# Elliotshui/ABRSimulator

Hardware: AMD Instinct MI355X
Metric: env_steps_per_sec (higher is better)
Workload: dtype f64

## Files before the change

### abrsimulator_amd/csrc/abr_env.hip

```cpp
#include <hip/hip_runtime.h>

#include <climits>
#include <cmath>
#include <cstdarg>
#include <cstdio>
#include <cstdlib>
#include <cstring>
#include <new>
#include <type_traits>
#include <vector>

#include "abr_env.h"

#ifdef ABR_SPLIT_STAMPS
#include "abr_diag_stamps.h"
#else
#define ABR_STAMP(n)
#define ABR_STAMP_INIT()
#define ABR_STAMP_FLUSH()
#define ABR_WG_TIME(slot)
#define ABR_WG_WHERE(role)
#define K3_STAMP_DECL
#define K3_STAMP(n)
#define K3_STAMP_FLUSH()
// ... 496 lines not shown
            const bool hit = dling && (dl2 >= target);
            done_dl = done_dl || hit;
            chunk_id += hit ? 1 : 0;
            avail_k = hit ? avail_next : avail_k;
            const double bufA = hit ? buf + L : buf;
            const bool playing = running && !(be || su);
            sk += playing ? (uint32_t)k : 0u;
            n_play += playing ? 1 : 0;
            const double bufB = playing ? bufA - sd : bufA;
            bf = bufB >= max_buffer;
            be = bufB <= 0.0;
            buf = be ? 0.0 : bufB;
            su = su && !(buf >= sul);
            k += running ? 1 : 0;
            const bool next = running && (chunk_id < V) && (k < max_ticks);
            n_su += (next && su) ? 1 : 0;
            n_rb += (next && !su && be) ? 1 : 0;
            const bool call = done_dl && (k >= avail_k) && !bf;
            running = next && !call;
            const bool cross = (k == k_end);
            c = cross ? c_next : c;
            crossed = crossed || cross;
        }
        if (active) {
            s.buf = buf; s.dl = dl; s.c = c; s.k = k; s.chunk_id = chunk_id; s.n_su = n_su;
            s.n_rb = n_rb; s.n_play = n_play; s.n_dl = n_dl; s.avail_k = avail_k;
            s.su = su; s.be = be; s.bf = bf; s.done_dl = done_dl; s.running = running;
            s.sumk += (long long)sk;
            (void)crossed;
        }
    }

    if (touched) {
        lane_store(s, p, i);
        p.n_su_obs[i] = n_su_obs; p.n_rb_obs[i] = n_rb_obs; p.episode_no[i] = episode_no;
        p.last_bw[i] = last_bw; p.hist_n[i] = hist_n; p.hist_s[i] = hist_s; p.var_run[i] = var_run;
        p.done[i] = done;
        if (MODE != 0) {
            for (int32_t t = step_idx; t < n_total; t++) {
                const int64_t o = (int64_t)t * p.n_lanes + i;
                if (reward_out) reward_out[o] = 0.0f;
                if (done_out) done_out[o] = done;
                if ((MODE == 2 || MODE == 4) && actions_out) actions_out[o] = -1;
                if (obs_out)
                    write_obs(s, p, i, obs_out + (int64_t)t * ABR_OBS_DIM * p.n_lanes, last_bw);
            }
        }
    }
}

using abrx::LaneJ;

template <bool SPEEDS>
struct SpeedParams;
template <>
struct SpeedParams<true> {
    static __device__ __forceinline__ const double *lane_speeds(const EnvParams &p) { return p.lane_speeds; }
    static __device__ __forceinline__ int32_t speed_rows(const EnvParams &p) { return p.speed_rows; }
    static __device__ __forceinline__ double *sd_lane(const EnvParams &p) { return p.sd_lane; }
    static __device__ __forceinline__ double *pt_lane(const EnvParams &p) { return p.pt_lane; }
    static __device__ __forceinline__ double *pt_sum(const EnvParams &p) { return p.pt_sum; }
    static __device__ __forceinline__ int32_t *pl_left(const EnvParams &p) { return p.pl_left; }
    static __device__ __forceinline__ int32_t *play_id(const EnvParams &p) { return p.play_id; }
};
template <>
struct SpeedParams<false> {
    static __device__ __forceinline__ constexpr const double *lane_speeds(const EnvParams &) { return nullptr; }
    static __device__ __forceinline__ constexpr int32_t speed_rows(const EnvParams &) { return 1; }
};

template <bool SPEEDS = true, class TB = abrx::TablesT<SPEEDS>>
__device__ inline TB make_tables(const EnvParams &p, bool cascade = true) {
    TB t;
    t.G = p.G; t.interval_tick = p.interval_tick; t.avail_tick = p.avail_tick;
    t.L = p.chunk_length; t.sd = p.sd; t.max_buffer = p.max_buffer;
    t.start_up_length = p.start_up_length; t.V = p.video_length; t.max_ticks = p.max_ticks;
    using SP = SpeedParams<SPEEDS>;
    if constexpr (SPEEDS) {
        t.per_lane_speed = SP::lane_speeds(p) != nullptr;
        t.speed_rows = SP::lane_speeds(p) ? SP::speed_rows(p) : 0;
        t.speed_stride = p.n_lanes; t.speeds = SP::lane_speeds(p);
    }
    t.drain = p.drain;
    if (SP::lane_speeds(p) || !cascade) t.drain.n = 0;
#ifdef ABR_NO_DRAIN_CASCADE
    t.drain.n = 0;
#endif
    return t;
}

template <bool SPEEDS = true>
__device__ inline void lanej_load(LaneJ &s, const EnvParams &p, int64_t i) {
    using SP = SpeedParams<SPEEDS>;
    s.buf = p.buf[i]; s.sumk = p.sumk[i];
    s.k = p.k[i]; s.chunk_id = p.chunk_id[i]; s.n_su = p.n_su[i]; s.n_rb = p.n_rb[i];
    s.n_play = p.n_play[i]; s.cur.j = p.j[i]; s.cur.tpos = p.tpos[i];
    s.last_action = p.last_action[i];
    const uint8_t f = p.flags[i];
    s.su = f & kFlagStartUp; s.be = f & kFlagBufEmpty; s.bf = f & kFlagBufFull;
    const int32_t c = s.chunk_id < p.video_length ? s.chunk_id : p.video_length;
    s.avail_k = p.avail_tick[c];
    if constexpr (SPEEDS) {
        if (SP::lane_speeds(p)) { s.sd = SP::sd_lane(p)[i]; s.pt = SP::pt_lane(p)[i]; } else { s.sd = p.sd; s.pt = 0.0; }
        s.lane = i; s.pl_left = 0; s.play_id = 0; s.pt_sum = 0.0;
        if (SP::lane_speeds(p) && SP::speed_rows(p) >= 2) { s.pl_left = SP::pl_left(p)[i]; s.play_id = SP::play_id(p)[i]; s.pt_sum = SP::pt_sum(p)[i]; }
    } else {
        s.sd = p.sd; s.lane = i;
    }
}

template <bool SPEEDS = true>
__device__ inline void lanej_store(const LaneJ &s, const EnvParams &p, int64_t i) {
    p.buf[i] = s.buf; p.sumk[i] = s.sumk;
    p.k[i] = s.k; p.chunk_id[i] = s.chunk_id; p.n_su[i] = s.n_su; p.n_rb[i] = s.n_rb;
    p.n_play[i] = s.n_play; p.j[i] = s.cur.j; p.tpos[i] = s.cur.tpos; p.last_action[i] = s.last_action;
    p.flags[i] = (uint8_t)((s.su ? kFlagStartUp : 0) | (s.be ? kFlagBufEmpty : 0) |
                           (s.bf ? kFlagBufFull : 0) | kFlagArmed);
    if constexpr (SPEEDS) {
        using SP = SpeedParams<SPEEDS>;
        if (SP::lane_speeds(p)) { SP::sd_lane(p)[i] = s.sd; SP::pt_lane(p)[i] = s.pt; }
        if (SP::lane_speeds(p) && SP::speed_rows(p) >= 2) { SP::pl_left(p)[i] = s.pl_left; SP::play_id(p)[i] = s.play_id; SP::pt_sum(p)[i] = s.pt_sum; }
    }
}

#ifndef ABR_NO_NT_STORES
#define ABR_OUT(ref, val) __builtin_nontemporal_store((val), &(ref))
#else
#define ABR_OUT(ref, val) ((ref) = (val))
#endif

template <bool SPEEDS = true>
__device__ inline void write_obs_j(const LaneJ &s, const EnvParams &p, int64_t i, float *obs,
                                   double last_bw) {
    if (!obs) return;
    const int64_t n = p.n_lanes;
    ABR_OUT(obs[ABR_OBS_CHUNK_ID * n + i], (float)s.chunk_id);
    ABR_OUT(obs[ABR_OBS_LAST_BITRATE * n + i], (float)s.last_action);
    ABR_OUT(obs[ABR_OBS_LAST_BANDWIDTH * n + i], (float)last_bw);
    ABR_OUT(obs[ABR_OBS_BUFFER_LEVEL * n + i], (float)s.buf);
    ABR_OUT(obs[ABR_OBS_GLOBAL_TIME * n + i], (float)p.G[s.k]);
    ABR_OUT(obs[ABR_OBS_PLAY_TIME * n + i], (float)(SpeedParams<SPEEDS>::lane_speeds(p) ? s.pt : p.GP[s.n_play]));
    ABR_OUT(obs[ABR_OBS_REBUFFER_TIME * n + i], (float)p.G[s.n_rb]);
    ABR_OUT(obs[ABR_OBS_STARTUP_TIME * n + i], (float)p.G[s.n_su]);
}

__device__ inline void write_obs_vals(const LaneJ &s, const EnvParams &p, int64_t i, float *obs, double last_bw,
                                      double g_k, double g_play, double g_rb, double g_su) {
    if (!obs) return;
    const int64_t n = p.n_lanes;
    ABR_OUT(obs[ABR_OBS_CHUNK_ID * n + i], (float)s.chunk_id);
    ABR_OUT(obs[ABR_OBS_LAST_BITRATE * n + i], (float)s.last_action);
    ABR_OUT(obs[ABR_OBS_LAST_BANDWIDTH * n + i], (float)last_bw);
    ABR_OUT(obs[ABR_OBS_BUFFER_LEVEL * n + i], (float)s.buf);
    ABR_OUT(obs[ABR_OBS_GLOBAL_TIME * n + i], (float)g_k);
    ABR_OUT(obs[ABR_OBS_PLAY_TIME * n + i], (float)g_play);
    ABR_OUT(obs[ABR_OBS_REBUFFER_TIME * n + i], (float)g_rb);
    ABR_OUT(obs[ABR_OBS_STARTUP_TIME * n + i], (float)g_su);
}

#ifndef ABR_JUMP_WAVES
#define ABR_JUMP_WAVES 5
#endif
#ifndef ABR_JUMP_WAVES_ONE
#define ABR_JUMP_WAVES_ONE 4
#endif
#define ABR_JUMP_BOUNDS(MODE, SAMPLE) \
// ... 288 lines not shown
    L->max_ticks = mt;
    L->n_intervals = (int32_t)n_iv;
    size_t o = 0;
    const size_t A = 256;
    size_t N = (size_t)n_lanes, V = (size_t)c->video_length;
    L->G = o; o = align_up(o + sizeof(double) * ((size_t)mt + 2), A);
    L->GP = o; o = align_up(o + sizeof(double) * ((size_t)mt + 2), A);
    L->interval_tick = o; o = align_up(o + sizeof(int32_t) * ((size_t)L->n_intervals + 8), A);
    L->avail_tick = o; o = align_up(o + sizeof(int32_t) * (V + 2), A);
    L->f64_state = o; o = align_up(o + sizeof(double) * 8 * N, A);
    L->i64_state = o; o = align_up(o + sizeof(long long) * 1 * N, A);
    L->i32_state = o; o = align_up(o + sizeof(int32_t) * 15 * N, A);
    L->u8_state = o; o = align_up(o + 2 * N, A);
    L->action_hist = o; o = align_up(o + V * N, A);
    L->bw_hist = o; o = align_up(o + sizeof(double) * V * N, A);
    L->ep_terms = o; o = align_up(o + sizeof(double) * 4 * N, A);
    L->mpc_action = o; o = align_up(o + sizeof(int32_t) * N, A);
    L->mpc_scratch = o; o = align_up(o + mpc_scratch_bytes_max(N), A);
    L->tag = o; o = align_up(o + sizeof(WorkspaceTag), A);
    L->total = o;
    return ABR_OK;
}

extern "C" int abr_env_workspace_bytes(const abr_env_config *cfg, int64_t n_lanes,
                                       size_t *bytes_out) {
    Layout L;
    int rc = compute_layout(cfg, n_lanes, &L);
    if (rc) return rc;
    if (!bytes_out) return fail(ABR_E_INVALID, "bytes_out is NULL");
    *bytes_out = L.total;
    return ABR_OK;
}

extern "C" int abr_env_create(const abr_env_config *cfg, const double *traces_dev,
                              const int64_t *trace_off_dev, const int32_t *trace_len_dev,
                              int32_t n_traces, int64_t n_lanes, void *workspace_dev,
                              size_t workspace_bytes, void *stream, abr_env **env_out) {
    Layout L;
    int rc = compute_layout(cfg, n_lanes, &L);
    if (rc) return rc;
    if (!env_out) return fail(ABR_E_INVALID, "env_out is NULL");
    if (!traces_dev || !trace_off_dev || !trace_len_dev || n_traces < 1)
        return fail(ABR_E_INVALID, "trace arrays missing");
    if (!workspace_dev || ((uintptr_t)workspace_dev & 255))
        return fail(ABR_E_WORKSPACE, "workspace must be non-NULL and 256-B aligned");
    if (workspace_bytes < L.total)
        return fail(ABR_E_WORKSPACE, "workspace has %zu bytes, need %zu", workspace_bytes, L.total);

    const int32_t mt = L.max_ticks;
    abrx::TickTables tt = abrx::build_tick_tables(cfg->interval, cfg->chunk_length, cfg->speed,
                                                  cfg->video_length, mt, L.n_intervals);
    std::vector<double> &G = tt.G, &GP = tt.GP;
    std::vector<int32_t> &itick = tt.interval_tick, &atick = tt.avail_tick;
    const double sd = tt.sd;
    const int32_t P = tt.play_ticks_per_chunk;
    int32_t t_block = tt.min_interval_ticks < 128 ? tt.min_interval_ticks : 128;
    if (t_block < 1) t_block = 1;
    if (P == INT_MAX)
        return fail(ABR_E_UNSUPPORTED, "max_ticks %d too small to play one chunk", mt);

    abr_env *e = new (std::nothrow) abr_env;
    if (!e) return fail(ABR_E_INVALID, "out of host memory");
    memset(e, 0, sizeof(*e));
    e->cfg = *cfg;
    e->impl = 3;
    e->chains_proven = abrx::chains_proven(itick.data(), itick.size(), mt, sd, cfg->chunk_length, cfg->max_buffer, cfg->ladder,
                                           cfg->n_rates);
    e->workspace_bytes = L.total;
    EnvParams &p = e->p;
    p.n_rates = cfg->n_rates; p.video_length = cfg->video_length; p.max_ticks = mt;
    p.auto_reset = cfg->auto_reset; p.play_ticks_per_chunk = P; p.n_intervals = L.n_intervals;
    p.t_block = t_block; p.n_traces = n_traces;
    p.chunk_length = cfg->chunk_length; p.max_buffer = cfg->max_buffer;
    p.start_up_length = cfg->start_up_length;
    p.wr = cfg->rebuffer_weight; p.wv = cfg->variance_weight; p.ws = cfg->startup_weight;
    p.wl = cfg->latency_weight; p.sd = sd;
    for (int r = 0; r < ABR_MAX_RATES; r++) p.ladder[r] = cfg->ladder[r];
    p.n_lanes = n_lanes; p.lane_id_base = 0;
    char *w = (char *)workspace_dev;
    p.G = (const double *)(w + L.G); p.GP = (const double *)(w + L.GP);
    p.interval_tick = (const int32_t *)(w + L.interval_tick);
    p.avail_tick = (const int32_t *)(w + L.avail_tick);
    p.drain = abrx::make_drain_tab(sd, cfg->max_buffer + cfg->chunk_length);
    p.traces = traces_dev; p.trace_off = trace_off_dev; p.trace_len = trace_len_dev;
    const size_t N = (size_t)n_lanes;
    double *f = (double *)(w + L.f64_state);
    p.buf = f; p.last_bw = f + N; p.hist_n = f + 2 * N; p.hist_s = f + 3 * N;
    p.sd_lane = f + 4 * N; p.pt_lane = f + 5 * N; p.pt_sum = f + 6 * N; p.var_run = f + 7 * N; p.lane_speeds = nullptr;
    p.speed_rows = 1;
    p.speed_rule = abrx::SpeedRuleBlock{};
    p.sumk = (long long *)(w + L.i64_state);
    int32_t *q = (int32_t *)(w + L.i32_state);
    p.k = q; p.chunk_id = q + N; p.n_su = q + 2 * N; p.n_rb = q + 3 * N; p.n_play = q + 4 * N;
    p.j = q + 5 * N; p.tpos = q + 6 * N; p.trace_id = q + 7 * N; p.offset0 = q + 8 * N;
    p.last_action = q + 9 * N; p.n_su_obs = q + 10 * N; p.n_rb_obs = q + 11 * N;
    p.episode_no = q + 12 * N; p.pl_left = q + 13 * N; p.play_id = q + 14 * N;
    uint8_t *u = (uint8_t *)(w + L.u8_state);
    p.flags = u; p.done = u + N;
    p.action_hist = (uint8_t *)(w + L.action_hist);
    p.bw_hist = (double *)(w + L.bw_hist);
    p.ep_qoe_terms = (double *)(w + L.ep_terms);
    e->mpc_action = (int32_t *)(w + L.mpc_action);
    e->mpc_scratch = (void *)(w + L.mpc_scratch);

    hipStream_t st = (hipStream_t)stream;
    hipError_t he;
#define UP(dst, vec)                                                                           \
    he = hipMemcpyAsync((void *)(dst), (vec).data(), (vec).size() * sizeof((vec)[0]),          \
                        hipMemcpyHostToDevice, st);                                            \
    if (he != hipSuccess) { delete e; return fail(ABR_E_HIP, "table upload: %s", hipGetErrorString(he)); }
    UP(p.G, G) UP(p.GP, GP) UP(p.interval_tick, itick) UP(p.avail_tick, atick)
#undef UP
    he = hipMemsetAsync(w + L.f64_state, 0, L.total - L.f64_state, st);
    if (he == hipSuccess) he = hipMemsetAsync(p.done, ABR_DONE_EPISODE, N, st);
    {
        WorkspaceTag &tg = e->tag;
        memset(&tg, 0, sizeof(tg));
        tg.magic = kTagMagic; tg.abi_version = ABR_ABI_VERSION; tg.layout_rev = kLayoutRev; tg.n_rates = (uint32_t)cfg->n_rates;
        tg.n_lanes = n_lanes; tg.video_length = cfg->video_length; tg.max_ticks = mt; tg.n_intervals = L.n_intervals;
        tg.total_bytes = L.total; tg.chunk_length = cfg->chunk_length; tg.interval = cfg->interval; tg.speed = cfg->speed;
        e->tag_dev = w + L.tag;
        if (he == hipSuccess) he = hipMemcpyAsync(e->tag_dev, &tg, sizeof(tg), hipMemcpyHostToDevice, st);
    }
    if (he == hipSuccess) he = hipStreamSynchronize(st);
    if (he != hipSuccess) { delete e; return fail(ABR_E_HIP, "workspace init: %s", hipGetErrorString(he)); }
    *env_out = e;
    return ABR_OK;
}

extern "C" int abr_env_destroy(abr_env *env) {
    delete env;
    return ABR_OK;
}

extern "C" int abr_env_has_impl(int32_t impl) {
    switch (impl) {
    case 0: case 1: case 2: case 3: case 5: return 1;
#ifdef ABR_WITH_ASYNC
    case 4: return 1;
#endif
#ifdef ABR_WITH_RING
    case 6: case 7: return 1;
#endif
    default: return 0;
    }
}

enum Feature { kLaneSpeeds, kSpeedRule, kRuleRollout, kMpcRollout, kPolicyRollout };
static const struct { unsigned impls; const char *what; } kFeatures[] = {
    {0xFDu, "per-lane speeds and speed schedules need the event-driven kernels"},
    {0x2Du, "a speed rule needs the event-driven kernels that read it"},
    {0x0Bu, "rule rollouts run on the one-thread-per-lane kernels"},
    {0xFDu, "the fused MPC rollout needs the event-driven kernels"},
    {0xFDu, "the fused policy rollout needs the event-driven kernels"},
};

static int require(Feature f, int impl) {
    const unsigned ok = kFeatures[f].impls;
    if (ok >> impl & 1u) return ABR_OK;
    int ks[8], n = 0, len = 0;
    for (int k = 0; k < 8; k++)
        if ((ok >> k & 1u) && abr_env_has_impl(k)) ks[n++] = k;
    char list[48] = "";
    for (int i = 0; i < n; i++)
        len += snprintf(list + len, sizeof(list) - len, "%s%d", i == 0 ? "" : i + 1 < n ? ", " : " or ", ks[i]);
    return fail(ABR_E_UNSUPPORTED, "%s (impl %s), not impl %d", kFeatures[f].what, list, impl);
// ... 3439 lines not shown
```

### abrsimulator_amd/csrc/abr_exact_jump.h

```cpp
#ifndef ABR_EXACT_JUMP_H
#define ABR_EXACT_JUMP_H

#include <stdint.h>
#include <string.h>

#if defined(__HIPCC__)
#define ABR_HD __host__ __device__ inline
#else
#define ABR_HD inline
#endif

namespace abrx {

ABR_HD int expo(double x) {
    uint64_t b;
#if defined(__HIP_DEVICE_COMPILE__)
    b = (uint64_t)__double_as_longlong(x);
#else
    memcpy(&b, &x, 8);
#endif
    return (int)((b >> 52) & 0x7ff);
}

ABR_HD double pow2_biased(int e) {
    uint64_t b = (uint64_t)e << 52;
    double r;
#if defined(__HIP_DEVICE_COMPILE__)
    r = __longlong_as_double((long long)b);
#else
    memcpy(&r, &b, 8);
#endif
    return r;
}

enum StopKind { STOP_GE = 0 , STOP_LE = 1 ,
                STOP_LT = 2  };

template <int STOP>
ABR_HD bool stop_hit(double x, double thr) {
    return STOP == STOP_GE ? (x >= thr) : (STOP == STOP_LE ? (x <= thr) : (x < thr));
}

ABR_HD double rcp_est(double d) {
#if defined(__HIP_DEVICE_COMPILE__)
    return __builtin_amdgcn_rcp(d);
#else
    return 1.0 / d;
#endif
}

ABR_HD int32_t sat_i32(double v) {
#if defined(__HIP_DEVICE_COMPILE__)
    int32_t r;
    asm("v_cvt_i32_f64 %0, %1" : "=v"(r) : "v"(v));
    return r;
#else
    if (!(v == v)) return 0;
    if (v >= 2147483647.0) return 2147483647;
    if (v <= -2147483648.0) return (-2147483647 - 1);
    return (int32_t)v;
#endif
}

struct ChainState {
    double x;
    int32_t eb;
};

ABR_HD double min_num(double a, double b) {
#if defined(__HIP_DEVICE_COMPILE__)
    double r;
    asm("v_min_f64 %0, %1, %2" : "=v"(r) : "v"(a), "v"(b));
    return r;
#else
    return (b < a) ? b : a;
#endif
}
ABR_HD double max_num(double a, double b) {
#if defined(__HIP_DEVICE_COMPILE__)
    double r;
    asm("v_max_f64 %0, %1, %2" : "=v"(r) : "v"(a), "v"(b));
    return r;
#else
    return (b > a) ? b : a;
#endif
}

template <int STOP>
ABR_HD bool jump_inside(double y, double lim, bool strict) {
    if (STOP == STOP_GE) return y < lim;
    return strict ? (y > lim) : (y >= lim);
}

constexpr int32_t kJumpCap = 1 << 20;

ABR_HD uint32_t clamp0(int32_t v, int32_t hi) {
#if defined(__HIP_DEVICE_COMPILE__)
    uint32_t r;
    asm("v_med3_i32 %0, %1, 0, %2" : "=v"(r) : "v"(v), "v"(hi));
    return r;
#else
    v = (v > 0) ? v : 0;
    return (uint32_t)((v < hi) ? v : hi);
#endif
}

ABR_HD double mul_add_u32(uint32_t q, double b, double a) {
#if defined(__HIP_DEVICE_COMPILE__)
    return __builtin_fma((double)q, b, a);
#else
    return a + (double)q * b;
#endif
}
ABR_HD double mul_sub_u32(uint32_t q, double b, double a) {
#if defined(__HIP_DEVICE_COMPILE__)
    return __builtin_fma(-(double)q, b, a);
#else
    return a - (double)q * b;
#endif
}

ABR_HD bool any_lane(bool v) {
#if defined(__HIP_DEVICE_COMPILE__)
    return __builtin_expect(__any(v) != 0, 0);
#else
    return v;
#endif
}

enum SettleKind { SETTLE_REMAINDER = 0, SETTLE_CANDIDATES = 1 };
enum GuardKind { GUARDS_CHECKED = 0, GUARDS_PROVEN = 1 };
template <int STOP, int BIAS = 0, int SETTLE = SETTLE_REMAINDER, int GUARDS = GUARDS_CHECKED>
ABR_HD int32_t chain_segment(ChainState &cs, double c, double thr, int32_t n_in, bool &hit_out) {
#ifdef ABR_SEGMENT_HOOK
    ABR_SEGMENT_HOOK(STOP);
#endif
    constexpr bool kProven = GUARDS == GUARDS_PROVEN;
#ifdef ABR_PROVEN_HOOK
    if (kProven) ABR_PROVEN_HOOK(STOP, n_in, cs.x);
#endif
    const int32_t n = (kProven || n_in < kJumpCap) ? n_in : kJumpCap;
    double x = cs.x;
    int32_t a = 0;
    const int e = expo(x);
    const bool normal = kProven | ((e > 54) & (e < 2046));
    const int ec = e;
    const double ac = (STOP == STOP_GE) ? c : -c;
    const double base = pow2_biased(ec);
    const double dm = (base + ac) - base;
    const double rem = ac - dm;
    const double half_u = base * 0x1p-53;
    const bool tie = ((rem < 0.0) ? -rem : rem) == half_u;
    const bool go = kProven | (n > 0);
    const int ea = expo(ac), ea_lo = (kProven && ea < 54) ? 54 : ea;
    const bool can = normal & go & (ea_lo < e) & (!tie | (cs.eb == e));
    const double d = (STOP == STOP_GE) ? dm : -dm;
    {
        double lim, gap;
        bool strict = true;
        if (STOP == STOP_GE) {
            lim = min_num(thr, base + base);
            gap = lim - x;
        } else {
            if (STOP == STOP_LE) {
                lim = max_num(thr, base);
            } else {
                strict = !(thr > base);
                lim = max_num(thr, base);
            }
            gap = x - lim;
        }
        const int32_t room = can ? n - 1 : 0;
        int32_t q0s = sat_i32(gap * rcp_est(dm));
        if (BIAS != 0) q0s = (q0s < 0x7fffff00 && q0s > -0x7fffff00) ? q0s + BIAS : q0s;
        const uint32_t q0 = clamp0(q0s, room);
        int32_t m, back;
        double xj;
        bool ok;
        if (SETTLE == SETTLE_REMAINDER) {
            const double r = mul_sub_u32(q0, dm, gap);
            bool longer, shorter;
            if (STOP == STOP_LT) {
                longer = strict ? (r > dm) : (r >= dm);
                shorter = strict ? (r <= 0.0) : (r < 0.0);
            } else {
                longer = r > dm;
                shorter = r <= 0.0;
            }
            m = (int32_t)clamp0((int32_t)q0 + (longer ? 1 : 0) - (shorter ? 1 : 0), room);
            xj = mul_add_u32((uint32_t)m, d, x);
            ok = (m == 0) | jump_inside<STOP>(xj, lim, strict);
            back = m;
        } else {
            const uint32_t bs = (q0 > 0) ? q0 - 1 : 0;
            const double y0 = x + (double)bs * d;
            const double y1 = y0 + d;
            const double y2 = y1 + d;
            const bool t1 = (bs + 1 <= (uint32_t)room) & jump_inside<STOP>(y1, lim, strict);
            const bool t2 = (bs + 2 <= (uint32_t)room) & jump_inside<STOP>(y2, lim, strict) & t1;
            m = (int32_t)(bs + (t1 ? 1 : 0) + (t2 ? 1 : 0));
            xj = t2 ? y2 : (t1 ? y1 : y0);
            ok = (bs == 0) | jump_inside<STOP>(y0, lim, strict);
            back = (int32_t)bs;
        }
#ifdef ABR_BRACKET_HOOK
        ABR_BRACKET_HOOK(ok);
#endif
        if (any_lane(!ok)) {
            int32_t mm = ok ? 0 : back;
#if defined(__HIP_DEVICE_COMPILE__)
#pragma clang loop unroll(disable) vectorize(disable)
#endif
            while (mm > 0 && !jump_inside<STOP>(x + (double)mm * d, lim, strict)) mm--;
            if (!ok) { m = mm; xj = x + (double)mm * d; }
        }
        x = xj;
        a = m;
    }
    const double xn = x + c;
    const bool hit = go & stop_hit<STOP>(xn, thr);
    x = go ? xn : x;
    a += go ? 1 : 0;
    cs.x = x;
    cs.eb = go ? e : cs.eb;
    hit_out = hit;
#ifdef ABR_SEGMENT_END_HOOK
    ABR_SEGMENT_END_HOOK(STOP, a, n_in, hit, can && expo(x) == e);
#endif
    return a;
}

template <int STOP, int BIAS = 0, int SETTLE = SETTLE_REMAINDER, int GUARDS = GUARDS_CHECKED>
ABR_HD bool chain(double &x_io, double c, double thr, int32_t n, int32_t &a_out) {
    ChainState cs;
    cs.x = x_io; cs.eb = -1;
    int32_t a = 0;
    bool hit = false;
    while (a < n && !hit) a += chain_segment<STOP, BIAS, SETTLE, GUARDS>(cs, c, thr, n - a, hit);
    x_io = cs.x;
    a_out = a;
    return hit;
}

struct DrainTab {
    int32_t e_hi = 0;
    int32_t n = 0;
    double top = 0.0;
    double rcp = 0.0;
};

ABR_HD bool wave_any(bool v) {
#if defined(__HIP_DEVICE_COMPILE__)
    return __any(v) != 0;
#else
    return v;
#endif
}

ABR_HD DrainTab make_drain_tab(double sd, double max_level) {
    DrainTab out;
    if (!(sd > 0.0) || !(max_level > 0.0) || !(sd < 1.0e300) || !(max_level < 1.0e300)) return out;
    const int es = expo(sd), eh = expo(max_level);
    if (es < 64 || es > 1900 || eh > 1900) return out;
    uint64_t bits;
#if defined(__HIP_DEVICE_COMPILE__)
    bits = (uint64_t)__double_as_longlong(sd);
#else
    memcpy(&bits, &sd, 8);
#endif
    const uint64_t mant = (bits & 0xfffffffffffffull) | (1ull << 52);
    int tz = 0;
    while (!((mant >> tz) & 1)) tz++;
    const int e_tie = es + 1 + tz;
    int e_lo = es + 2;
    if (e_tie >= e_lo && e_tie <= eh) e_lo = e_tie + 1;
    if (e_lo > eh) return out;
    if (eh - e_lo + 1 > 64) return out;
    if (pow2_biased(eh) * 2.0 / sd >= 67108864.0) return out;
    if (pow2_biased(e_lo) * 2.0 / sd > 64.0) return out;
    out.e_hi = eh; out.n = eh - e_lo + 1;
    out.top = pow2_biased(eh) * 2.0;
    out.rcp = 1.0 / sd;
    return out;
}

ABR_HD bool drain_cascade(const DrainTab &tb_in, double sd, double &x_io, int32_t m, int32_t &a_out) {
    int32_t tb_n = tb_in.n, tb_e_hi = tb_in.e_hi;
    double tb_rcp = tb_in.rcp;
#if defined(__HIP_DEVICE_COMPILE__)
    asm volatile("" : "+v"(sd), "+v"(tb_rcp), "+v"(tb_n), "+v"(tb_e_hi));
    tb_n = __builtin_amdgcn_readfirstlane(tb_n);
    tb_e_hi = __builtin_amdgcn_readfirstlane(tb_e_hi);
#endif
    double x = x_io;
    int32_t a = 0;
    int32_t i = 0;
#if defined(__HIP_DEVICE_COMPILE__)
#pragma unroll 1
#endif
    while (i < tb_n && !wave_any((a < m) & (x >= pow2_biased(tb_e_hi - i)))) i++;
#if defined(__HIP_DEVICE_COMPILE__)
#pragma unroll 1
#endif
    for (; i < tb_n && wave_any(a < m); i++) {
        const int e = tb_e_hi - i;
        const double base = pow2_biased(e);
        const double u = pow2_biased(e - 52);
        const double S = (base + sd) - base;
        const double T = (S >= sd) ? S : S + u;
        const double B = base + T;
        const double g = x - B;
        int32_t q = sat_i32(g * tb_rcp);
        const double r = g - (double)q * S;
        q -= (r < 0.0) ? 1 : 0;
        q += (r >= S) ? 1 : 0;
        int32_t n = q + 1;
        const int32_t left = m - a;
        n = n < left ? n : left;
        n = n > 0 ? n : 0;
        x = x - (double)n * S;
        a += n;
// ... 18 lines not shown
```

### abrsimulator_amd/csrc/abr_lane_jump.h

```cpp
#ifndef ABR_LANE_JUMP_H
#define ABR_LANE_JUMP_H

#include <math.h>

#include "abr_exact_jump.h"

#ifndef ABR_STAMP
#define ABR_STAMP(n)
#endif

namespace abrx {

constexpr double kTickDt = 0.01;
#ifndef ABR_K_DRAIN_TAIL
#define ABR_K_DRAIN_TAIL 16
#endif
constexpr int kPrologue = 16;
#ifndef ABR_PCHUNKS
#define ABR_PCHUNKS 12
#endif
#ifndef ABR_PCHECK
#define ABR_PCHECK 0x892
#endif
constexpr int kPChunks = ABR_PCHUNKS;
constexpr int kPCheck = ABR_PCHECK;

struct SpeedRule {
    int32_t n_lat, n_buf;
    double lat_thr[4], buf_thr[4];
    double speed[5][5];
};

ABR_HD double speed_rule_eval(const SpeedRule &r, double lat, double buf) {
    int32_t i = 0, j = 0;
    for (int32_t q = 0; q < r.n_lat; q++) i += lat >= r.lat_thr[q] ? 1 : 0;
    for (int32_t q = 0; q < r.n_buf; q++) j += buf >= r.buf_thr[q] ? 1 : 0;
    return r.speed[i][j];
}

constexpr int32_t kSpeedRowsRule = 0x7fffffff;

struct SpeedRuleBlock {
    SpeedRule rule;
    double *log;
    int32_t log_rows, reserved_;
};

template <bool SPEEDS = true>
struct TablesT;

template <>
struct TablesT<true> {
    static constexpr bool kSpeeds = true;
    static constexpr int kSettle = SETTLE_REMAINDER;
    static constexpr int kGuards = GUARDS_CHECKED;
    const double *G;
    const int32_t *interval_tick;
    const int32_t *avail_tick;
    double L, sd, max_buffer, start_up_length;
    int32_t V, max_ticks;
    bool per_lane_speed;
    int32_t speed_rows;
    int64_t speed_stride;
    const double *speeds;
    const SpeedRuleBlock *rule = nullptr;
    DrainTab drain;
};

template <>
struct TablesT<false> {
    static constexpr bool kSpeeds = false;
    static constexpr int kSettle = SETTLE_REMAINDER;
    static constexpr int kGuards = GUARDS_PROVEN;
    const double *G;
    const int32_t *interval_tick;
    const int32_t *avail_tick;
    double L, sd, max_buffer, start_up_length;
    int32_t V, max_ticks;
    static constexpr bool per_lane_speed = false;
    static constexpr int32_t speed_rows = 0;
    static constexpr int64_t speed_stride = 0;
    static constexpr const double *speeds = nullptr;
    static constexpr const SpeedRuleBlock *rule = nullptr;
    DrainTab drain;
};

using Tables = TablesT<true>;

struct TablesCandidates : TablesT<true> {
    static constexpr int kSettle = SETTLE_CANDIDATES;
};

struct TablesChecked : TablesT<false> {
    static constexpr int kGuards = GUARDS_CHECKED;
};

inline bool chains_proven(const int32_t *interval_tick, size_t n_interval_tick, int32_t max_ticks, double sd,
                          double chunk_length, double max_buffer, const double *ladder, int32_t n_rates) {
    if (max_ticks < 1 || max_ticks > kJumpCap) return false;
    for (size_t j = 0; j + 1 < n_interval_tick && interval_tick[j] != 0x7fffffff; j++) {
        if (interval_tick[j + 1] == 0x7fffffff) break;
        const int64_t span = (int64_t)interval_tick[j + 1] - interval_tick[j];
        if (span < 1 || span >= kJumpCap) return false;
    }
    const auto bounded = [](double v) { return v == v && v > -0x1p960 && v < 0x1p960; };
    if (!bounded(sd) || !bounded(chunk_length) || !bounded(max_buffer)) return false;
    for (int32_t r = 0; r < n_rates; r++)
        if (!bounded(ladder[r] * chunk_length)) return false;
    return true;
}

struct Cursor {
    int32_t j;
    int32_t tpos;
    int32_t tlen;
    const double *trace;
};

struct LaneJ {
    double buf;
    double sd;
    double pt;
    long long sumk;
    int32_t k, chunk_id, n_su, n_rb, n_play, avail_k, last_action;
    bool su, be, bf;
    Cursor cur;
    int32_t pl_left, play_id;
    double pt_sum;
    int64_t lane;
};

ABR_HD void cursor_init(Cursor &c, int32_t offset0) {
    c.j = 0;
    c.tpos = offset0 % c.tlen;
}

template <class TB>
ABR_HD void lanej_init_player(LaneJ &s, const TB &t) {
    s.buf = 0.0; s.sumk = 0;
    s.k = 0; s.chunk_id = 0; s.n_su = 1; s.n_rb = 0; s.n_play = 0;
    s.last_action = -1;
    s.su = true; s.be = true; s.bf = false;
    s.avail_k = t.avail_tick[0];
    if constexpr (TB::kSpeeds) {
        s.pt = 0.0;
        s.pl_left = 0; s.play_id = 0; s.pt_sum = 0.0;
    }
}

template <class TB>
ABR_HD void lanej_init(LaneJ &s, const TB &t, int32_t offset0) {
    lanej_init_player(s, t);
    cursor_init(s.cur, offset0);
}

template <class TB>
ABR_HD void lanej_play(LaneJ &s, const TB &t, int32_t a) {
    if (!t.per_lane_speed || a <= 0) return;
    int32_t done = 0;
    double x = s.pt;
    chain<STOP_GE, 0, TB::kSettle, TB::kGuards>(x, s.sd, 1.0e300, a, done);
    s.pt = x;
}

constexpr int kDrainTail = ABR_K_DRAIN_TAIL;
template <int SETTLE = SETTLE_REMAINDER, int GUARDS = GUARDS_CHECKED>
ABR_HD bool drain_to_zero(double &b_io, double sd, int32_t m, int32_t &a_out) {
    ChainState cs;
    cs.x = b_io; cs.eb = -1;
    const double tail = (double)kDrainTail * sd;
    int32_t a = 0;
    bool below = false;
    while (a < m && !below) a += chain_segment<STOP_LE, 0, SETTLE, GUARDS>(cs, -sd, tail, m - a, below);
    double b = cs.x;
    ABR_STAMP(24);
#ifdef ABR_DRAIN_HOOK
    const int32_t a_seg = a;
#endif
#if defined(__HIP_DEVICE_COMPILE__)
#pragma unroll 1
#endif
    while (a < m && b > 0.0) { b = b - sd; a++; }
    ABR_STAMP(25);
#ifdef ABR_DRAIN_HOOK
    ABR_DRAIN_HOOK(a > 0 && b <= 0.0, a - a_seg);
#endif
    b_io = b; a_out = a;
    return a > 0 && b <= 0.0;
}

template <class TB>
ABR_HD bool lanej_drain(const TB &t, double &b_io, double sd, int32_t m, int32_t &a_out) {
    if (t.drain.n > 0 && !wave_any(!(b_io < t.drain.top))) {
        const bool zero = drain_cascade(t.drain, sd, b_io, m, a_out);
        ABR_STAMP(24);
        return zero;
    }
    return drain_to_zero<TB::kSettle, TB::kGuards>(b_io, sd, m, a_out);
}

template <class TB>
ABR_HD void sched_begin_chunk(LaneJ &s, const TB &t, int32_t k, double b) {
    double v;
    if (t.speed_rows == kSpeedRowsRule) {
#if defined(__HIP_DEVICE_COMPILE__) && defined(ABR_RULE_KERNARG_OFFSET)
        auto kp = __builtin_amdgcn_kernarg_segment_ptr();
        asm volatile("" : "+s"(kp));
        const SpeedRuleBlock &rb = *(const SpeedRuleBlock *)((const char *)kp + ABR_RULE_KERNARG_OFFSET);
#else
        const SpeedRuleBlock &rb = *t.rule;
#endif
        v = speed_rule_eval(rb.rule, t.G[k] - s.pt, b);
        if (s.play_id < rb.log_rows) rb.log[(int64_t)s.play_id * t.speed_stride + s.lane] = v;
    } else {
        const int32_t row = s.play_id < t.speed_rows ? s.play_id : t.speed_rows - 1;
        v = t.speeds[(int64_t)row * t.speed_stride + s.lane];
    }
    s.sd = v * kTickDt;
    double x = 0.0;
    int32_t a = 0;
    chain<STOP_GE, 0, TB::kSettle, TB::kGuards>(x, s.sd, t.L, t.max_ticks + 1, a);
    s.pl_left = a > 0 ? a : 1;
}

template <class TB>
ABR_HD void sched_played(LaneJ &s, const TB &t, int32_t a) {
    if (a <= 0) return;
    s.pt_sum += (double)a * s.pt + s.sd * (double)(((long long)a * (a - 1)) / 2);
    int32_t done = 0;
    double x = s.pt;
    chain<STOP_GE, 0, TB::kSettle, TB::kGuards>(x, s.sd, 1.0e300, a, done);
    s.pt = x;
    s.pl_left -= a;
    if (s.pl_left == 0) s.play_id++;
}

template <int STOP, class TB>
ABR_HD bool sched_drain(LaneJ &s, const TB &t, double &b, double thr, int32_t m, int32_t &a_out) {
    int32_t a_tot = 0;
    bool hit = false;
    while (a_tot < m && !hit) {
        if (s.pl_left == 0) sched_begin_chunk(s, t, s.k + a_tot, b);
        const int32_t run = (m - a_tot < s.pl_left) ? m - a_tot : s.pl_left;
        int32_t a = 0;
        if (STOP == STOP_LE) hit = drain_to_zero<TB::kSettle, TB::kGuards>(b, s.sd, run, a);
        else hit = chain<STOP_LT, 0, TB::kSettle, TB::kGuards>(b, -s.sd, thr, run, a);
        sched_played(s, t, a);
        a_tot += a;
    }
    a_out = a_tot;
    return hit;
}

template <class TB>
ABR_HD void lanej_idle(LaneJ &s, const TB &t, int32_t m) {
    if (m <= 0) return;
    if (s.su && s.buf >= t.start_up_length) s.su = false;
    ABR_STAMP(23);
    if (s.su) {
        s.n_su += m;
    } else if (s.be) {
        s.n_rb += m;
    } else {
        int32_t a = 0;
        double b = s.buf;
        bool zero;
        if constexpr (TB::kSpeeds) {
            if (t.speed_rows >= 2) zero = sched_drain<STOP_LE>(s, t, b, 0.0, m, a);
            else { zero = lanej_drain(t, b, s.sd, m, a); lanej_play(s, t, a); }
        } else {
            zero = lanej_drain(t, b, t.sd, m, a);
        }
        s.n_play += a;
        s.sumk += (long long)a * s.k + ((long long)a * (a - 1)) / 2;
        if (zero) { b = 0.0; s.be = true; s.n_rb += (m - a + 1); }
        s.buf = b;
        s.bf = b >= t.max_buffer;
    }
    s.k += m;
}

template <class TB>
ABR_HD bool lanej_wait_call(LaneJ &s, const TB &t) {
    const int32_t mt = t.max_ticks;
    if (s.k >= s.avail_k && !s.bf) return true;
    int32_t w = s.avail_k - s.k;
    if (w < 0) w = 0;
    if (w > mt - s.k) w = mt - s.k;
    lanej_idle(s, t, w);
    if (s.k >= mt) return false;
    if (s.bf) {
        if (s.su || s.be) {
            if (s.su) s.n_su += mt - s.k; else s.n_rb += mt - s.k;
            s.k = mt;
            return false;
        }
        int32_t a = 0;
        double b = s.buf;
        bool cleared;
        if constexpr (TB::kSpeeds) {
            if (t.speed_rows >= 2) cleared = sched_drain<STOP_LT>(s, t, b, t.max_buffer, mt - s.k, a);
            else { cleared = chain<STOP_LT, 0, TB::kSettle, TB::kGuards>(b, -s.sd, t.max_buffer, mt - s.k, a); lanej_play(s, t, a); }
        } else {
            cleared = chain<STOP_LT, 0, TB::kSettle, TB::kGuards>(b, -t.sd, t.max_buffer, mt - s.k, a);
        }
        s.n_play += a;
        s.sumk += (long long)a * s.k + ((long long)a * (a - 1)) / 2;
        s.k += a;
        s.be = b <= 0.0;
        if (s.be) { b = 0.0; s.n_rb += 1; }
        s.buf = b;
        s.bf = !cleared;
        if (!cleared) return false;
    }
    return true;
}

struct StepResult {
    double bw;
    bool hit;
    bool ended;
    bool timeout;
};

constexpr int kCatch = 4;
struct StepStart {
    double c;
    double bw_next;
    int32_t ke;
    int32_t ke_next;
    int32_t tn;
    int32_t avail_next;
};

ABR_HD int32_t trace_wrap(int32_t pos, int32_t tlen) {
    if (pos >= tlen) pos -= tlen;
    if (pos >= tlen) pos %= tlen;
    return pos;
}

struct StepLoads {
    int32_t ke[kCatch + 2];
    double bw[kCatch + 2];
    int32_t avail_next;
};

template <class TB>
ABR_HD StepLoads lanej_begin_load(const Cursor &s, const TB &t, int32_t chunk_id) {
    StepLoads ld;
#if defined(__HIP_DEVICE_COMPILE__)
#pragma unroll
#endif
    for (int i = 0; i < kCatch + 2; i++) {
        ld.ke[i] = t.interval_tick[s.j + 1 + i];
        ld.bw[i] = s.trace[trace_wrap(s.tpos + i, s.tlen)];
    }
    ld.avail_next = t.avail_tick[chunk_id + 1];
    return ld;
}

template <class TB>
ABR_HD StepStart lanej_begin_select(Cursor &s, const TB &t, const StepLoads &ld, int32_t k) {
    const int32_t *ke = ld.ke;
    const double *bw = ld.bw;
    StepStart st;
    st.avail_next = ld.avail_next;
    int32_t adv = 0;
#if defined(__HIP_DEVICE_COMPILE__)
#pragma unroll
#endif
    for (int i = 0; i < kCatch; i++) adv += (k >= ke[i]) ? 1 : 0;
    if (adv == kCatch && k >= ke[kCatch]) {
        s.j += kCatch; s.tpos = trace_wrap(s.tpos + kCatch, s.tlen);
        int32_t e = t.interval_tick[s.j + 1];
        while (k >= e && e != 0x7fffffff) {
            s.j++;
            s.tpos = (s.tpos + 1 == s.tlen) ? 0 : s.tpos + 1;
            e = t.interval_tick[s.j + 1];
        }
        st.ke = e; st.ke_next = t.interval_tick[s.j + 2];
        st.tn = (s.tpos + 1 == s.tlen) ? 0 : s.tpos + 1;
        st.c = s.trace[s.tpos] * kTickDt; st.bw_next = s.trace[st.tn];
        return st;
    }
    double c_bw = bw[0], n_bw = bw[1];
    int32_t c_ke = ke[0], n_ke = ke[1];
#if defined(__HIP_DEVICE_COMPILE__)
// ... 84 lines not shown
    Download d;
    d.dl = cs.x; d.n_dl = kk - k; d.hit = hit;
    return d;
}

template <class TB>
ABR_HD StepResult lanej_after_download(LaneJ &s, const TB &t, const Download &d,
                                       int32_t avail_next, int32_t action) {
    StepResult r;
    r.bw = 0.0; r.hit = false; r.ended = false; r.timeout = false;
    const int32_t mt = t.max_ticks;
    const bool hit = d.hit;
    const int32_t n_dl = d.n_dl;
    const double g_ndl = t.G[n_dl];
    lanej_idle(s, t, hit ? n_dl - 1 : n_dl);
    ABR_STAMP(10);
    if (!hit) { r.timeout = true; return r; }
    const bool playing = !(s.be || s.su);
    double b = s.buf + t.L;
    if (playing) {
        s.sumk += s.k; s.n_play++;
        if constexpr (TB::kSpeeds) {
            if (t.speed_rows >= 2) {
                if (s.pl_left == 0) sched_begin_chunk(s, t, s.k, b);
                b = b - s.sd;
                sched_played(s, t, 1);
            } else { b = b - s.sd; lanej_play(s, t, 1); }
        } else {
            b = b - t.sd;
        }
    }
    s.bf = b >= t.max_buffer;
    s.be = b <= 0.0;
    if (s.be) b = 0.0;
    s.buf = b;
    s.su = s.su && !(b >= t.start_up_length);
    s.k++;
    r.hit = true;
    r.bw = d.dl / g_ndl;
    s.last_action = action;
    s.chunk_id++;
    s.avail_k = avail_next;
    r.ended = s.chunk_id >= t.V;
    r.timeout = !r.ended && s.k >= mt;
    ABR_STAMP(11);
    if (!r.ended && !r.timeout) {
        s.n_su += s.su ? 1 : 0;
        s.n_rb += (!s.su && s.be) ? 1 : 0;
        r.timeout = !lanej_wait_call(s, t);
    }
    ABR_STAMP(12);
    return r;
}

template <class TB>
ABR_HD bool lanej_gate_possible(double buf, bool su, bool be, int32_t n_dl, const TB &t) {
    return !su && !be && !t.per_lane_speed && (buf + t.L) - (double)n_dl * t.sd >= t.max_buffer - 1.0e-6;
}
template <class TB>
ABR_HD bool lanej_predict_next_call(double buf, int32_t k, int32_t n_dl, int32_t avail_next, const TB &t,
                                    int32_t &k_next, double *buf_next = nullptr) {
    const int32_t mt = t.max_ticks;
    double b = buf;
    int32_t a = 0;
    if (n_dl > 1 && lanej_drain(t, b, t.sd, n_dl - 1, a)) return false;
    b = b + t.L;
    b = b - t.sd;
    if (b <= 0.0) return false;
    bool bf = b >= t.max_buffer;
    k += n_dl;
    if (k >= mt) return false;
    if (!(k >= avail_next && !bf)) {
        int32_t w = avail_next - k;
        if (w < 0) w = 0;
        if (w > mt - k) w = mt - k;
        if (w > 0) {
            if (lanej_drain(t, b, t.sd, w, a)) return false;
            bf = b >= t.max_buffer;
            k += w;
        }
        if (k >= mt) return false;
        if (bf) {
            a = 0;
            if (!chain<STOP_LT, 0, TB::kSettle, TB::kGuards>(b, -t.sd, t.max_buffer, mt - k, a)) return false;
            k += a;
            if (b <= 0.0) return false;
        }
    }
    k_next = k;
    if (buf_next) *buf_next = b;
    return true;
}

template <class TB>
ABR_HD StepResult lanej_download_and_wait(LaneJ &s, const TB &t, const StepStart &st,
                                          double target, int32_t action) {
    const Download d = lanej_download(s.cur, t, st, s.k, target);
    return lanej_after_download(s, t, d, st.avail_next, action);
}

template <class TB>
ABR_HD StepResult lanej_step(LaneJ &s, const TB &t, double target, int32_t action) {
    const StepStart st = lanej_begin_step(s.cur, t, s.k, s.chunk_id);
    return lanej_download_and_wait(s, t, st, target, action);
}

enum { kRuleBuffer = 1, kRuleRate = 2, kRuleBola = 3, kRuleFastMpc = 4 };

struct RuleParams {
    int32_t kind, window;
    double reservoir, cushion;
    double safety;
    double bola_v, bola_gp;
    const double *utility;
    const uint8_t *fm_table;
    int32_t fm_uniform;
    int32_t fm_horizon, fm_nb, fm_nq;
};

template <class BR>
ABR_HD int32_t rule_hi(const BR &br, int32_t M, double X) {
    int32_t a = 0;
    for (int32_t m = 1; m < M; m++) a = br(m) <= X ? m : a;
    return a;
}

template <class BR>
ABR_HD int32_t rule_buffer(const RuleParams &r, const BR &br, int32_t M, double B) {
    if (B <= r.reservoir) return 0;
    if (B >= r.reservoir + r.cushion) return M - 1;
    const double lo = br(0);
    return rule_hi(br, M, lo + ((B - r.reservoir) / r.cushion) * (br(M - 1) - lo));
}

template <class HIST>
ABR_HD double harmonic_tail(const HIST &hist, int32_t c, int32_t n) {
    double S = 0.0;
    for (int32_t j = c - n; j < c; j++) S = S + 1.0 / hist(j);
    return (double)n / S;
}

template <class BR, class HIST>
ABR_HD int32_t rule_rate(const RuleParams &r, const BR &br, const HIST &hist, int32_t M, int32_t c) {
    const int32_t n = r.window < c ? r.window : c;
    if (n <= 0) return 0;
    return rule_hi(br, M, r.safety * harmonic_tail(hist, c, n));
}

template <class BR>
ABR_HD int32_t rule_bola(const RuleParams &r, const BR &br, int32_t M, int32_t c, double B) {
    const double *u = r.utility + (int64_t)c * M;
    double best = (r.bola_v * (u[0] + r.bola_gp) - B) / br(0);
    int32_t a = 0;
    for (int32_t m = 1; m < M; m++) {
        const double sc = (r.bola_v * (u[m] + r.bola_gp) - B) / br(m);
        a = sc > best ? m : a;
        best = sc > best ? sc : best;
    }
    return a;
}

template <class BR, class HIST>
ABR_HD int32_t rule_select(const RuleParams &r, const BR &br, const HIST &hist, int32_t M, int32_t c, double B) {
    if (r.kind == kRuleBuffer) return rule_buffer(r, br, M, B);
    if (r.kind == kRuleRate) return rule_rate(r, br, hist, M, c);
    return rule_bola(r, br, M, c, B);
}
// ... 1028 lines not shown
```

Measured before the change: 13.67 billion.

## Use precomputed reciprocal of drain rate and flat asm drain tail in proven tables

Adds a host-precomputed 1/sd to the drain table and, for the proven no-speed table type, passes it into chain_segment in place of the per-segment rcp_est(dm). The proof condition chains_proven is extended with a range check on that reciprocal. It also replaces the scalar drain tail loop with an inline-asm, exec-masked unrolled sequence of tick decrements and raises the tail length from 16 to 24. The aim is to cut reciprocal estimation and divergent loop overhead, at the cost of more fixed tail instructions per drain and hand-written assembly.

```diff
diff --git a/abrsimulator_amd/csrc/abr_env.hip b/abrsimulator_amd/csrc/abr_env.hip
--- a/abrsimulator_amd/csrc/abr_env.hip
+++ b/abrsimulator_amd/csrc/abr_env.hip
@@ -602,6 +602,7 @@
         t.speed_stride = p.n_lanes; t.speeds = SP::lane_speeds(p);
     }
     t.drain = p.drain;
+    if constexpr (!SPEEDS) t.rsd = p.drain.rcp;
     if (SP::lane_speeds(p) || !cascade) t.drain.n = 0;
 #ifdef ABR_NO_DRAIN_CASCADE
     t.drain.n = 0;
@@ -1056,6 +1057,8 @@
     p.interval_tick = (const int32_t *)(w + L.interval_tick);
     p.avail_tick = (const int32_t *)(w + L.avail_tick);
     p.drain = abrx::make_drain_tab(sd, cfg->max_buffer + cfg->chunk_length);
+    p.drain.rcp = 1.0 / sd;
+    e->chains_proven = e->chains_proven && abrx::rcp_proven(sd, cfg->max_buffer + cfg->chunk_length);
     p.traces = traces_dev; p.trace_off = trace_off_dev; p.trace_len = trace_len_dev;
     const size_t N = (size_t)n_lanes;
     double *f = (double *)(w + L.f64_state);
diff --git a/abrsimulator_amd/csrc/abr_exact_jump.h b/abrsimulator_amd/csrc/abr_exact_jump.h
--- a/abrsimulator_amd/csrc/abr_exact_jump.h
+++ b/abrsimulator_amd/csrc/abr_exact_jump.h
@@ -94,6 +94,10 @@
 
 constexpr int32_t kJumpCap = 1 << 20;
 
+inline bool rcp_proven(double sd, double max_level) {
+    return sd >= 0x1p-1000 && sd < 0x1p960 && max_level == max_level && max_level / sd < 0x1p25;
+}
+
 ABR_HD uint32_t clamp0(int32_t v, int32_t hi) {
 #if defined(__HIP_DEVICE_COMPILE__)
     uint32_t r;
@@ -130,8 +134,8 @@
 
 enum SettleKind { SETTLE_REMAINDER = 0, SETTLE_CANDIDATES = 1 };
 enum GuardKind { GUARDS_CHECKED = 0, GUARDS_PROVEN = 1 };
-template <int STOP, int BIAS = 0, int SETTLE = SETTLE_REMAINDER, int GUARDS = GUARDS_CHECKED>
-ABR_HD int32_t chain_segment(ChainState &cs, double c, double thr, int32_t n_in, bool &hit_out) {
+template <int STOP, int BIAS = 0, int SETTLE = SETTLE_REMAINDER, int GUARDS = GUARDS_CHECKED, bool RCP = false>
+ABR_HD int32_t chain_segment(ChainState &cs, double c, double thr, int32_t n_in, bool &hit_out, double rcp = 0.0) {
 #ifdef ABR_SEGMENT_HOOK
     ABR_SEGMENT_HOOK(STOP);
 #endif
@@ -171,7 +175,7 @@
             gap = x - lim;
         }
         const int32_t room = can ? n - 1 : 0;
-        int32_t q0s = sat_i32(gap * rcp_est(dm));
+        int32_t q0s = sat_i32(gap * (RCP ? rcp : rcp_est(dm)));
         if (BIAS != 0) q0s = (q0s < 0x7fffff00 && q0s > -0x7fffff00) ? q0s + BIAS : q0s;
         const uint32_t q0 = clamp0(q0s, room);
         int32_t m, back;
@@ -230,13 +234,13 @@
     return a;
 }
 
-template <int STOP, int BIAS = 0, int SETTLE = SETTLE_REMAINDER, int GUARDS = GUARDS_CHECKED>
-ABR_HD bool chain(double &x_io, double c, double thr, int32_t n, int32_t &a_out) {
+template <int STOP, int BIAS = 0, int SETTLE = SETTLE_REMAINDER, int GUARDS = GUARDS_CHECKED, bool RCP = false>
+ABR_HD bool chain(double &x_io, double c, double thr, int32_t n, int32_t &a_out, double rcp = 0.0) {
     ChainState cs;
     cs.x = x_io; cs.eb = -1;
     int32_t a = 0;
     bool hit = false;
-    while (a < n && !hit) a += chain_segment<STOP, BIAS, SETTLE, GUARDS>(cs, c, thr, n - a, hit);
+    while (a < n && !hit) a += chain_segment<STOP, BIAS, SETTLE, GUARDS, RCP>(cs, c, thr, n - a, hit, rcp);
     x_io = cs.x;
     a_out = a;
     return hit;
diff --git a/abrsimulator_amd/csrc/abr_lane_jump.h b/abrsimulator_amd/csrc/abr_lane_jump.h
--- a/abrsimulator_amd/csrc/abr_lane_jump.h
+++ b/abrsimulator_amd/csrc/abr_lane_jump.h
@@ -13,7 +13,7 @@
 
 constexpr double kTickDt = 0.01;
 #ifndef ABR_K_DRAIN_TAIL
-#define ABR_K_DRAIN_TAIL 16
+#define ABR_K_DRAIN_TAIL 24
 #endif
 constexpr int kPrologue = 16;
 #ifndef ABR_PCHUNKS
@@ -54,6 +54,8 @@
     static constexpr bool kSpeeds = true;
     static constexpr int kSettle = SETTLE_REMAINDER;
     static constexpr int kGuards = GUARDS_CHECKED;
+    static constexpr bool kRcp = false;
+    static constexpr bool kFlatTail = false;
     const double *G;
     const int32_t *interval_tick;
     const int32_t *avail_tick;
@@ -72,10 +74,17 @@
     static constexpr bool kSpeeds = false;
     static constexpr int kSettle = SETTLE_REMAINDER;
     static constexpr int kGuards = GUARDS_PROVEN;
+#ifdef ABR_NO_TABLE_RCP
+    static constexpr bool kRcp = false;
+#else
+    static constexpr bool kRcp = true;
+#endif
+    static constexpr bool kFlatTail = true;
     const double *G;
     const int32_t *interval_tick;
     const int32_t *avail_tick;
     double L, sd, max_buffer, start_up_length;
+    double rsd = 0.0;
     int32_t V, max_ticks;
     static constexpr bool per_lane_speed = false;
     static constexpr int32_t speed_rows = 0;
@@ -93,7 +102,21 @@
 
 struct TablesChecked : TablesT<false> {
     static constexpr int kGuards = GUARDS_CHECKED;
-};
+    static constexpr bool kRcp = false;
+    static constexpr bool kFlatTail = false;
+};
+
+template <class TB>
+ABR_HD double table_rsd(const TB &t) {
+    if constexpr (TB::kRcp) {
+#if !defined(__HIP_DEVICE_COMPILE__)
+        if (t.rsd == 0.0) return 1.0 / t.sd;
+#endif
+        return t.rsd;
+    } else {
+        return 0.0;
+    }
+}
 
 inline bool chains_proven(const int32_t *interval_tick, size_t n_interval_tick, int32_t max_ticks, double sd,
                           double chunk_length, double max_buffer, const double *ladder, int32_t n_rates) {
@@ -164,23 +187,91 @@
 }
 
 constexpr int kDrainTail = ABR_K_DRAIN_TAIL;
-template <int SETTLE = SETTLE_REMAINDER, int GUARDS = GUARDS_CHECKED>
-ABR_HD bool drain_to_zero(double &b_io, double sd, int32_t m, int32_t &a_out) {
+#ifndef ABR_DRAIN_TAIL_FORM
+#define ABR_DRAIN_TAIL_FORM 2
+#endif
+
+ABR_HD void drain_tail_ticks(double &b, int32_t &a, double sd, int32_t m) {
+#if defined(__HIP_DEVICE_COMPILE__) && ABR_DRAIN_TAIL_FORM == 2
+    uint64_t saved;
+#define ABR_TAIL_TICK "v_cmpx_lt_f64 vcc, 0, %[b]\n\tv_add_f64 %[b], %[b], -%[sd]\n\tv_add_u32 %[a], 1, %[a]\n\tv_cmpx_lt_i32 vcc, %[a], %[m]\n\t"
+#define ABR_TAIL_TICKS4 ABR_TAIL_TICK ABR_TAIL_TICK ABR_TAIL_TICK ABR_TAIL_TICK "s_cbranch_execz .Labr_tail_end_%=\n\t"
+    static_assert(kDrainTail % 4 == 0 && kDrainTail >= 4 && kDrainTail <= 32, "the tail is unrolled four ticks at a time");
+    asm volatile("s_mov_b64 %[saved], exec\n\t"
+                 "v_cmpx_lt_i32 vcc, %[a], %[m]\n\t"
+                 ABR_TAIL_TICKS4
+#if ABR_K_DRAIN_TAIL >= 8
+                 ABR_TAIL_TICKS4
+#endif
+#if ABR_K_DRAIN_TAIL >= 12
+                 ABR_TAIL_TICKS4
+#endif
+#if ABR_K_DRAIN_TAIL >= 16
+                 ABR_TAIL_TICKS4
+#endif
+#if ABR_K_DRAIN_TAIL >= 20
+                 ABR_TAIL_TICKS4
+#endif
+#if ABR_K_DRAIN_TAIL >= 24
+                 ABR_TAIL_TICKS4
+#endif
+#if ABR_K_DRAIN_TAIL >= 28
+                 ABR_TAIL_TICKS4
+#endif
+#if ABR_K_DRAIN_TAIL >= 32
+                 ABR_TAIL_TICKS4
+#endif
+                 ".Labr_tail_end_%=:\n\t"
+                 "s_mov_b64 exec, %[saved]"
+                 : [b] "+v"(b), [a] "+v"(a), [saved] "=&s"(saved)
+                 : [sd] "v"(sd), [m] "v"(m)
+                 : "vcc");
+#undef ABR_TAIL_TICKS4
+#undef ABR_TAIL_TICK
+#else
+#if defined(__HIP_DEVICE_COMPILE__)
+#pragma unroll
+#endif
+    for (int i = 0; i < kDrainTail; i++) {
+        const bool go = (a < m) & (b > 0.0);
+        b = go ? b - sd : b;
+        a += go ? 1 : 0;
+    }
+#endif
+}
+
+template <int SETTLE = SETTLE_REMAINDER, int GUARDS = GUARDS_CHECKED, bool RCP = false, bool FLAT = false>
+ABR_HD bool drain_to_zero(double &b_io, double sd, int32_t m, int32_t &a_out, double rsd = 0.0) {
     ChainState cs;
     cs.x = b_io; cs.eb = -1;
     const double tail = (double)kDrainTail * sd;
     int32_t a = 0;
     bool below = false;
-    while (a < m && !below) a += chain_segment<STOP_LE, 0, SETTLE, GUARDS>(cs, -sd, tail, m - a, below);
+    while (a < m && !below) a += chain_segment<STOP_LE, 0, SETTLE, GUARDS, RCP>(cs, -sd, tail, m - a, below, rsd);
     double b = cs.x;
     ABR_STAMP(24);
 #ifdef ABR_DRAIN_HOOK
     const int32_t a_seg = a;
 #endif
+    if (FLAT && ABR_DRAIN_TAIL_FORM != 0) {
+        if (wave_any((a < m) & (b > 0.0))) {
+            drain_tail_ticks(b, a, sd, m);
+#ifdef ABR_DRAIN_LEFT_HOOK
+            ABR_DRAIN_LEFT_HOOK(a < m && b > 0.0);
+#endif
+            if (any_lane((a < m) & (b > 0.0))) {
 #if defined(__HIP_DEVICE_COMPILE__)
 #pragma unroll 1
 #endif
-    while (a < m && b > 0.0) { b = b - sd; a++; }
+                while (a < m && b > 0.0) { b = b - sd; a++; }
+            }
+        }
+    } else {
+#if defined(__HIP_DEVICE_COMPILE__)
+#pragma unroll 1
+#endif
+        while (a < m && b > 0.0) { b = b - sd; a++; }
+    }
     ABR_STAMP(25);
 #ifdef ABR_DRAIN_HOOK
     ABR_DRAIN_HOOK(a > 0 && b <= 0.0, a - a_seg);
@@ -196,7 +287,7 @@
         ABR_STAMP(24);
         return zero;
     }
-    return drain_to_zero<TB::kSettle, TB::kGuards>(b_io, sd, m, a_out);
+    return drain_to_zero<TB::kSettle, TB::kGuards, TB::kRcp, TB::kFlatTail>(b_io, sd, m, a_out, table_rsd(t));
 }
 
 template <class TB>
@@ -302,7 +393,7 @@
             if (t.speed_rows >= 2) cleared = sched_drain<STOP_LT>(s, t, b, t.max_buffer, mt - s.k, a);
             else { cleared = chain<STOP_LT, 0, TB::kSettle, TB::kGuards>(b, -s.sd, t.max_buffer, mt - s.k, a); lanej_play(s, t, a); }
         } else {
-            cleared = chain<STOP_LT, 0, TB::kSettle, TB::kGuards>(b, -t.sd, t.max_buffer, mt - s.k, a);
+            cleared = chain<STOP_LT, 0, TB::kSettle, TB::kGuards, TB::kRcp>(b, -t.sd, t.max_buffer, mt - s.k, a, table_rsd(t));
         }
         s.n_play += a;
         s.sumk += (long long)a * s.k + ((long long)a * (a - 1)) / 2;
@@ -553,7 +644,7 @@
         if (k >= mt) return false;
         if (bf) {
             a = 0;
-            if (!chain<STOP_LT, 0, TB::kSettle, TB::kGuards>(b, -t.sd, t.max_buffer, mt - k, a)) return false;
+            if (!chain<STOP_LT, 0, TB::kSettle, TB::kGuards, TB::kRcp>(b, -t.sd, t.max_buffer, mt - k, a, table_rsd(t))) return false;
             k += a;
             if (b <= 0.0) return false;
         }
```

New measurement: 13.83 billion, median of 3. About the same (+1.2%).
